# igilitschenski/multi_car_racing

Hardware: AMD Instinct MI355X
Metric: env-steps/sec (num_agents=2, 96x96 RGB obs) at batch=4096; 1 GPU (higher is better)
Workload: dtype f32 rigid-body state / f64 tyre model / u8 pixels

## Files before the change

### include/mcr.h

```cpp
#ifndef MCR_H
#define MCR_H
#include <stddef.h>
#include <stdint.h>
#ifdef __cplusplus
extern "C" {
#endif

#define MCR_OK 0
#define MCR_ERR_ARG (-1)
#define MCR_ERR_HIP (-2)
#define MCR_ERR_STATE (-3)
#define MCR_ERR_CAPACITY (-4)

#define MCR_MAX_AGENTS 8
#define MCR_TILE_CAP 512
#define MCR_QUAD_CAP 768
#define MCR_OBS_H 96
#define MCR_OBS_W 96
#define MCR_MT_WORDS 625
#define MCR_OBS_RGB 0
#define MCR_OBS_GRAY 1
#define MCR_OBS_STACK_MAX 8

typedef struct mcr_env mcr_env;
// ... 140 lines not shown
int mcr_debug_read_view_scratch(mcr_env* h, int view, void* out, int nbytes);
int mcr_debug_read_dynamics_stamps(mcr_env* h, uint64_t* out, int n_u64);
int mcr_debug_read_counters(mcr_env* h, uint64_t* out4);
int mcr_debug_read_counters8(mcr_env* h, uint64_t* out8);
int mcr_debug_read_verdict_mismatches(mcr_env* h, uint64_t* out1);
int mcr_concurrent_collide(const mcr_env* h);
int mcr_step_ordering(const mcr_env* h);
int mcr_step_ordering_for(const mcr_env* h, void* stream);
int mcr_bind_stream(mcr_env* h, void* stream);
int mcr_debug_read_env_records(mcr_env* h, void* out, int n_bytes);
int mcr_debug_read_partition(mcr_env* h, uint8_t* part_out, int32_t* clist_out);
int mcr_debug_next_verdicts(mcr_env* h, int fill_value, uint8_t* out_or_null);
int mcr_debug_read_contact_counts(mcr_env* h, int32_t* out );
int mcr_debug_read_contacts(mcr_env* h, uint32_t* out );
int mcr_debug_read_tile_touch(mcr_env* h, uint32_t* out );
int mcr_debug_read_proxy_ids(mcr_env* h, int env, int32_t* out, int cap);
int mcr_status(mcr_env* h, uint32_t* out, int n_words);
int mcr_debug_overlap(mcr_env* h, int n, const float* quads, const float* poses, int fixture, uint8_t* out);
int mcr_debug_level_stats(const uint8_t* d_done, const uint8_t* d_trunc ,
                          const double* d_ep_return , const int32_t* d_ep_len,
                          const int32_t* d_level, int num_envs, int num_agents, int K,
                          int32_t* d_finished , double* d_stats , void* stream);
int mcr_debug_contact_obs(const uint32_t* d_store, int num_envs, int num_agents, int accumulate,
                          int32_t* d_mask , double* d_impulse , void* stream);
#define MCR_TIMING_SLOTS 8
int mcr_timing_read(mcr_env* h, double* ms_out , int64_t* launches_out );

#ifdef __cplusplus
}
#endif
// ... 2 lines not shown
```

### multi_car_racing_amd/_lib.py

```python
import ctypes, os
import numpy as np

HERE = os.path.dirname(os.path.abspath(__file__))
LIB_PATH = os.environ.get("MCR_LIB_PATH") or os.path.join(HERE, "_lib", "libmcr_hip.so")

MAX_AGENTS = 8
TILE_CAP = 512
QUAD_CAP = 768
MT_WORDS = 625
OBS_RGB, OBS_GRAY, OBS_STACK_MAX = 0, 1, 8
REPEAT_MAX = 16
RANGE_RAYS_MAX = 32
GRID_MAX = 64
GRID_ROAD, GRID_FRESH, GRID_TAKEN, GRID_CAR = 1, 2, 4, 8
DRV_PARAMS = 10
DRIVER_PARAM_NAMES = ("L1", "L2", "v_max", "K_s", "K_c", "K_g", "K_b", "offset", "gas_max", "brake_max")
DRIVER_DEFAULTS = dict(zip(DRIVER_PARAM_NAMES, (4.0, 12.0, 70.0, 8.0, 20.0, 0.2, 0.1, 0.0, 1.0, 0.8)))
RC_PARAMS = 8
RACECRAFT_PARAM_NAMES = ("look", "w_block", "w_pass", "off_max", "d_safe", "K_f", "w_off", "v_off")
RACECRAFT_DEFAULTS = dict(zip(RACECRAFT_PARAM_NAMES, (24.0, 3.5, 4.25, 4.5, 16.0, 2.0, 7.5, 15.0)))
LEVEL_ORDER = {"random": 0, "cycle": 1}

DEBUG_VIEW_CLOCKS = 1 << 5
DEBUG_POS_ITERS_2 = 1 << 6
# ... 94 lines not shown
    "mcr_hull_polygons": (_i, [_vp, _vp]),
    "mcr_driver_defaults": (_i, [_vp]),
    "mcr_check_drivers": (_i, [_i, _vp, ctypes.c_uint32]),
    "mcr_set_drivers": (_i, [_vp, _vp, ctypes.c_uint32, _vp]),
    "mcr_driver_actions": (_i, [_vp, _vp, ctypes.c_uint32, _vp, _vp]),
    "mcr_racecraft_defaults": (_i, [_vp]),
    "mcr_check_racecraft": (_i, [_i, _vp, ctypes.c_uint32]),
    "mcr_set_racecraft": (_i, [_vp, _vp, ctypes.c_uint32]),
    "mcr_read_rollout_stats": (_i, [_vp, _vp, _i]),
    "mcr_render": (_i, [_vp, _i, _i, _i, _vp, _vp]),
    "mcr_debug_read_contact_counts": (_i, [_vp, _vp]),
    "mcr_debug_read_contacts": (_i, [_vp, _vp]),
    "mcr_debug_contact_obs": (_i, [_vp, _i, _i, _i, _vp, _vp, _vp]),
    "mcr_debug_read_tile_touch": (_i, [_vp, _vp]),
    "mcr_debug_read_proxy_ids": (_i, [_vp, _i, _vp, _i]),
    "mcr_debug_read_env_records": (_i, [_vp, _vp, _i]),
    "mcr_debug_read_partition": (_i, [_vp, _vp, _vp]),
    "mcr_debug_next_verdicts": (_i, [_vp, _i, _vp]),
    "mcr_debug_read_counters": (_i, [_vp, _vp]),
    "mcr_debug_read_counters8": (_i, [_vp, _vp]),
    "mcr_debug_read_verdict_mismatches": (_i, [_vp, _vp]),
    "mcr_concurrent_collide": (_i, [_vp]),
    "mcr_step_ordering": (_i, [_vp]),
    "mcr_step_ordering_for": (_i, [_vp, _vp]),
    "mcr_bind_stream": (_i, [_vp, _vp]),
    "mcr_debug_overlap": (_i, [_vp, _i, _vp, _vp, _i, _vp]),
    "mcr_debug_level_stats": (_i, [_vp, _vp, _vp, _vp, _vp, _i, _i, _i, _vp, _vp, _vp]),
    "mcr_status": (_i, [_vp, _vp, _i]),
    "mcr_world_create": (_vp, [_i]),
    "mcr_world_destroy": (None, [_vp]),
# ... 103 lines not shown
```

### multi_car_racing_amd/csrc/k_carview.h

```cpp
#pragma once
#include "mcr_kernels.h"

struct CarPose {
  float cx[5], cy[5], a[5];
  float hvx, hvy, hw;
  double omega[4], phase[4];
};
#define CARVIEW_ALL 31u
struct CarBox { float xl, yl, xh, yh; };

__device__ __forceinline__ CarPose car_pose_load(const float* __restrict__ carf, const double* __restrict__ card, const int stride, const int ci, const uint32_t parts) {
  CarPose c = {};
#pragma unroll
  for (int k = 0; k < 5; ++k) {
    const bool mine = (parts >> k) & 1u;
    if (mine) { c.cx[k] = carf[(CF_CX + k) * stride + ci]; c.cy[k] = carf[(CF_CY + k) * stride + ci]; }
    if (mine || (k == 1 && (parts & 1u))) c.a[k] = carf[(CF_A + k) * stride + ci];
    if (mine && k > 0) c.phase[k - 1] = card[(CD_PHASE + k - 1) * stride + ci];
  }
  if (parts & 1u) {
    c.hvx = carf[(CF_VX + 0) * stride + ci]; c.hvy = carf[(CF_VY + 0) * stride + ci]; c.hw = carf[(CF_W + 0) * stride + ci];
#pragma unroll
    for (int k = 0; k < 4; ++k) c.omega[k] = card[(CD_OMEGA + k) * stride + ci];
  }
  return c;
}
__device__ __forceinline__ void car_pose_store(float* __restrict__ carf, double* __restrict__ card, const int stride, const int ci, const CarPose& c) {
#pragma unroll
  for (int k = 0; k < 5; ++k) { carf[(CF_CX + k) * stride + ci] = c.cx[k]; carf[(CF_CY + k) * stride + ci] = c.cy[k]; carf[(CF_A + k) * stride + ci] = c.a[k]; }
  carf[(CF_VX + 0) * stride + ci] = c.hvx; carf[(CF_VY + 0) * stride + ci] = c.hvy; carf[(CF_W + 0) * stride + ci] = c.hw;
#pragma unroll
  for (int k = 0; k < 4; ++k) { card[(CD_OMEGA + k) * stride + ci] = c.omega[k]; card[(CD_PHASE + k) * stride + ci] = c.phase[k]; }
}

__device__ __forceinline__ void view_score(float* __restrict__ vp, const double reward_shown, const uint32_t flags) {
  vp[VP_SCORE] = __int_as_float(mcr_label_value(reward_shown));
  vp[VP_OLDFLAGS] = __uint_as_float(flags);
}

__device__ __forceinline__ void carbox_add(CarBox& box, const V2 v) {
// ... 21 lines not shown
    double s1, s2, c1, c2; mcr_sincos_core(a1, &s1, &c1); mcr_sincos_core(a2, &s2, &c2);
    int ns = 0;
    if (!(s1 > 0 && s2 > 0)) {
      if (s1 > 0) c1 = np_sign(c1);
      if (s2 > 0) c2 = np_sign(c2);
      ns = 4;
      const float lx[4] = {(float)(-MCR_WHEEL_W * MCR_SIZE), (float)(+MCR_WHEEL_W * MCR_SIZE), (float)(+MCR_WHEEL_W * MCR_SIZE), (float)(-MCR_WHEEL_W * MCR_SIZE)};
      const float ly[4] = {(float)(+MCR_WHEEL_R * c1 * MCR_SIZE), (float)(+MCR_WHEEL_R * c1 * MCR_SIZE), (float)(+MCR_WHEEL_R * c2 * MCR_SIZE), (float)(+MCR_WHEEL_R * c2 * MCR_SIZE)};
      V2 u[4];
#pragma unroll
      for (int i = 0; i < 4; ++i) u[i] = xmul(wxf, v2(lx[i], ly[i]));
      carpoly_quad(cp4 + (2 * k + 1) * 4, u);
    }
    *(float2*)(cnt + 2 * k) = make_float2(__int_as_float(S.wheel.n), __int_as_float(ns));
  }
  if (parts & 1u) {
    const Xf hxf = xf_of(v2(c.cx[0], c.cy[0]), c.a[0], v2(S.hull_lcx, S.hull_lcy));
    const double zoom = 0.1 * MCR_SCALE * fmax(1 - t, 0.0) + MCR_ZOOM * MCR_SCALE * fmin(t, 1.0);
    const double sx = (double)hxf.p.x, sy = (double)hxf.p.y;
    double angle = -(double)c.a[0];
    const double vx = (double)c.hvx, vy = (double)c.hvy;
    const double speed = sqrt(vx * vx + vy * vy);
    if (speed > 0.5) angle = atan2(vx, vy);
    double sin_a, cos_a; mcr_sincos_core(angle, &sin_a, &cos_a);
    const double ttx = MCR_WINDOW_W / 2 - (sx * zoom * cos_a - sy * zoom * sin_a);
    const double tty = MCR_WINDOW_H * h_ratio - (sx * zoom * sin_a + sy * zoom * cos_a);
    const float ftx = (float)ttx, fty = (float)tty, fz = (float)zoom;
    const float fdeg = (float)(57.29577951308232 * angle);
    const double rad = (double)fdeg * (3.14159265358979323846 / 180.0);
    double sin_r, cos_r; mcr_sincos_core(rad, &sin_r, &cos_r);
    const float fcs = (float)cos_r, fsn = (float)sin_r;
    const float kx = 96.0f / 1000.0f, ky = 96.0f / 800.0f;
    vp[VP_CAM + 0] = fcs * fz * kx; vp[VP_CAM + 1] = -fsn * fz * kx; vp[VP_CAM + 2] = fsn * fz * ky; vp[VP_CAM + 3] = fcs * fz * ky;
    vp[VP_CAM + 4] = ftx * kx; vp[VP_CAM + 5] = fty * ky;
    const float inv_z = 1.0f / fz;
    const float i0 = fcs * (1000.0f / 96.0f) * inv_z, i1 = fsn * (800.0f / 96.0f) * inv_z, i2 = -(fcs * ftx + fsn * fty) * inv_z;
    const float i3 = -fsn * (1000.0f / 96.0f) * inv_z, i4 = fcs * (800.0f / 96.0f) * inv_z, i5 = (fsn * ftx - fcs * fty) * inv_z;
    vp[VP_INV + 0] = i0; vp[VP_INV + 1] = i1; vp[VP_INV + 2] = i2; vp[VP_INV + 3] = i3; vp[VP_INV + 4] = i4; vp[VP_INV + 5] = i5;
    const double sW = MCR_WINDOW_W / 40.0, hH = MCR_WINDOW_H / 40.0;
    const double vals[5] = {0.02 * speed, 0.01 * c.omega[0], 0.01 * c.omega[1], 0.01 * c.omega[2], 0.01 * c.omega[3]};
    const double places[5] = {5, 7, 8, 9, 10};
    float hud_top = 12.0f;
#pragma unroll
    for (int i = 0; i < 5; ++i) {
      const float ya = (float)(hH + hH * vals[i]) * ky, yb = (float)hH * ky;
      vp[VP_IND + i * 4 + 0] = (float)((places[i] + 0) * sW) * kx; vp[VP_IND + i * 4 + 1] = (float)((places[i] + 1) * sW) * kx;
      vp[VP_IND + i * 4 + 2] = fminf(ya, yb); vp[VP_IND + i * 4 + 3] = fmaxf(ya, yb);
      hud_top = fmaxf(hud_top, fmaxf(ya, yb) + 1.0f);
    }
    const double jang = (double)(c.a[1] - c.a[0]);
    const double hv[2] = {-10.0 * jang, -0.8 * (double)c.hw};
    const double hp[2] = {20, 30};
#pragma unroll
    for (int i = 0; i < 2; ++i) {
      const float xa = (float)((hp[i] + 0) * sW) * kx, xb = (float)((hp[i] + hv[i]) * sW) * kx;
      vp[VP_IND + (5 + i) * 4 + 0] = fminf(xa, xb); vp[VP_IND + (5 + i) * 4 + 1] = fmaxf(xa, xb);
      vp[VP_IND + (5 + i) * 4 + 2] = (float)(2 * hH) * ky; vp[VP_IND + (5 + i) * 4 + 3] = (float)(4 * hH) * ky;
    }
    vp[VP_HUDTOP] = hud_top;
    {
      const float hk = 0.5f / (float)(MCR_PLAYFIELD / 20.0);
      const float aU = i0 * hk, bU = i1 * hk, cU = i2 * hk;
      const float aV = i3 * hk, bV = i4 * hk, cV = i5 * hk;
      float umin = MCR_MAXFLT, umax = -MCR_MAXFLT, vmin = MCR_MAXFLT, vmax = -MCR_MAXFLT;
#pragma unroll
      for (int k = 0; k < 4; ++k) {
        const float X = (k & 1) ? 96.0f : 0.0f, Y = (k & 2) ? 96.0f : 12.0f;
        const float u = aU * X + bU * Y + cU, v = aV * X + bV * Y + cV;
        umin = fminf(umin, u); umax = fmaxf(umax, u); vmin = fminf(vmin, v); vmax = fmaxf(vmax, v);
      }
      const float mu = fabsf(aU) + fabsf(bU) + 1e-3f, mv = fabsf(aV) + fabsf(bV) + 1e-3f;
      const bool inside_field = umin - mu >= -10.0f && umax + mu <= 10.0f && vmin - mv >= -10.0f && vmax + mv <= 10.0f;
      int a0 = (int)ceilf(umin - mu - 0.5f), a1 = (int)floorf(umax + mu), b0 = (int)ceilf(vmin - mv - 0.5f), b1 = (int)floorf(vmax + mv);
      a0 = max(a0, -10); a1 = min(a1, 9); b0 = max(b0, -10); b1 = min(b1, 9);
      vp[VP_GRASS + 0] = __int_as_float(a0); vp[VP_GRASS + 1] = __int_as_float(max(a1 - a0 + 1, 0));
      vp[VP_GRASS + 2] = __int_as_float(b0); vp[VP_GRASS + 3] = __int_as_float(max(b1 - b0 + 1, 0));
      vp[VP_GRASS + 4] = __int_as_float(inside_field ? 1 : 0);
    }
    int hn[4];
#pragma unroll
    for (int k = 0; k < 4; ++k) {
      const int n = hn[k] = __builtin_amdgcn_readfirstlane(S.hull[k].n);
      V2 w[8];
#pragma unroll
      for (int i = 0; i < 8; ++i) { if (i < n) w[i] = xmul(hxf, v2(S.hull[k].vx[i], S.hull[k].vy[i])); else w[i] = w[i - 1 < 0 ? 0 : i - 1]; }
#pragma unroll
      for (int i = 0; i < 8; ++i) carbox_add(box, w[i]);
      float4* hp4 = cp4 + (8 + k) * 4;
#pragma unroll
      for (int i = 0; i < 4; ++i) hp4[i] = make_float4(w[2 * i].x, w[2 * i].y, w[2 * i + 1].x, w[2 * i + 1].y);
    }
    *(float4*)(cnt + 8) = make_float4(__int_as_float(hn[0]), __int_as_float(hn[1]), __int_as_float(hn[2]), __int_as_float(hn[3]));
  }
  return box;
}
```

### multi_car_racing_amd/csrc/k_list_chain.h

```cpp
#pragma once
#include "k_collide.h"
#include "k_dynamics.h"
#include "k_flags.h"
#include "k_viewprep.h"

__device__ __forceinline__ void list_reset_pass(const McrParams& p, const int blk) {
  __threadfence();
  if (p.term_idx) for (int k = 0; k < p.list_envs_per_block; ++k) term_prepare(p, mcr_env_of_slot(p, blk * p.list_envs_per_block + k));
  for (int k = 0; k < p.list_envs_per_block; ++k) { collide_block(p, 1, blk * p.list_envs_per_block + k); __syncthreads(); }
  __threadfence();
  __syncthreads();
  dynamics_block<true>(p, 1, blk);
  __syncthreads();
}

template <bool CC>
__global__ __launch_bounds__(64) void k_list_chain(McrParams pa, McrParams pb, const int with_flags, const int ga) {
  __builtin_amdgcn_s_setprio(3);
  if (pa.role == ROLE_CONTACT && blockIdx.x == 0 && threadIdx.x == 0) __hip_atomic_store(&pa.host_counts[HC_CONTACT_ENVS], (uint32_t)pa.clist[0], __ATOMIC_RELAXED, __HIP_MEMORY_SCOPE_SYSTEM);
  if (pa.soft_sync && pa.role == ROLE_DEFERRED && pa.cc_mode) {
    if (threadIdx.x == 0) (void)mcr_await(pa, W_COL);
    __builtin_amdgcn_fence(__ATOMIC_ACQUIRE, "agent");
    __syncthreads();
  }
// ... 40 lines not shown
  for (int blk = blockIdx.x; blk < nb; blk += gridDim.x) flags_block(p, blk);
}

__global__ void k_term_finish(McrParams p) { term_finish(p); }
__global__ __launch_bounds__(64) void k_term_prep(McrParams p) { term_prepare(p, p.env0 + (int)blockIdx.x); }

__global__ void k_post(McrParams p, int w) {
  if (threadIdx.x == 0 && w == W_SIDE && p.fuse_collide) p.clist[0] = 0;
  if (threadIdx.x == 0 && !((p.debug & DEBUG_NO_SIDE_POST) && w == W_SIDE)) mcr_post(p, w);
}
__global__ void k_await(McrParams p, int w0, int w1) {
  if (threadIdx.x == 0) { if (w0 >= 0) (void)mcr_await(p, w0); if (w1 >= 0) (void)mcr_await(p, w1); }
}

__global__ __launch_bounds__(64) void k_viewprep_verdict(McrParams p, const int vp_blocks) {
  if ((int)blockIdx.x < vp_blocks) { viewprep_block(p, (int)blockIdx.x); return; }
  if (p.part_next == nullptr) return;
  const int env = mcr_env_of_slot(p, (int)blockIdx.x - vp_blocks);
  if (env >= p.env0 + p.nenv || p.part_next[env] != 2) return;
  verdict_block(p, env);
}
__global__ __launch_bounds__(64, 8) void k_flags_viewprep(McrParams p, const int vp_blocks) {
  if ((int)blockIdx.x < vp_blocks) viewprep_block(p, (int)blockIdx.x);
  else flags_block(p, (int)blockIdx.x - vp_blocks);
}
```

### multi_car_racing_amd/csrc/k_viewprep.h

```cpp
#pragma once
#include "k_carview.h"

__device__ __forceinline__ void viewprep_car(const McrShapes& S, const float* __restrict__ carf, const double* __restrict__ card, const int stride, const int ci,
                                             float* __restrict__ viewp, float* __restrict__ carpoly, const double h_ratio, const double t_now, const uint32_t parts = CARVIEW_ALL) {
  view_record(S, car_pose_load(carf, card, stride, ci, parts), t_now, h_ratio, viewp + (size_t)ci * MCR_VIEWP_FLOATS, carpoly + (size_t)ci * MCR_CARPOLY_FLOATS, parts);
}

__device__ __forceinline__ void viewprep_block(const McrParams& p, const int blk) {
  const int g = blk * 64 + threadIdx.x;
  const int env = mcr_env_of_slot(p, g / p.G), agent = g % p.G;
  if (env >= p.env0 + p.nenv || agent >= p.N) return;
  const McrEnvState es = p.env[env];
  if (!es.active || es.just_reset) return;
  viewprep_car(*p.shapes, p.carf, p.card, p.BN, env * p.N + agent, p.viewp, p.carpoly, p.h_ratio, es.t);
}
__device__ __forceinline__ void viewprep_list_block(const McrParams& p, const int blk) {
  if (p.obs == nullptr) return;
  __builtin_amdgcn_fence(__ATOMIC_SEQ_CST, "workgroup");
  const int lane = threadIdx.x & 63, ncars = p.list_envs_per_block * p.N;
  for (int base = 0; base < ncars * 8; base += 64) {
    const int w = base + lane, c = w >> 3, part = w & 7;
    if (c >= ncars || part >= 5) continue;
    const int env = mcr_env_of_slot(p, blk * p.list_envs_per_block + c / p.N);
    if (env >= p.env0 + p.nenv) continue;
    const McrEnvState es = p.env[env];
    if (!es.active || es.resetting) continue;
    viewprep_car(*p.shapes, p.carf, p.card, p.BN, env * p.N + c % p.N, p.viewp, p.carpoly, p.h_ratio, es.t, 1u << part);
  }
}
__device__ __forceinline__ void term_prepare(const McrParams& p, const int env) {
  if (p.term_idx == nullptr || env >= p.env0 + p.nenv) return;
  const McrEnvState es = p.env[env];
  if (!es.active || !es.resetting) return;
  const int tidx = p.term_idx[env];
  if (tidx < 0) return;
  const int lane = threadIdx.x & 63;
  const uint32_t* __restrict__ src = (const uint32_t*)(p.tile_flags + (size_t)env * MCR_TILE_CAP);
  uint32_t* __restrict__ dst = (uint32_t*)(p.term_tflags + (size_t)tidx * MCR_TILE_CAP);
  for (int i = lane; i < MCR_TILE_CAP / 2; i += 64) dst[i] = src[i];
  if (lane < p.N) viewprep_car(*p.shapes, p.term_carf, p.term_card, p.term_cap * p.N, tidx * p.N + lane, p.term_viewp, p.term_carpoly, p.h_ratio, p.term_env[tidx].t);
}
__global__ __launch_bounds__(64) void k_viewprep(McrParams p) { viewprep_block(p, (int)blockIdx.x); }
__global__ __launch_bounds__(64) void k_viewprep_now(McrParams p) {
  const int ci = (int)blockIdx.x * 64 + (int)threadIdx.x;
  if (ci >= p.BN) return;
  const McrEnvState es = p.env[ci / p.N];
  if (!es.active) return;
  viewprep_car(*p.shapes, p.carf, p.card, p.BN, ci, p.viewp, p.carpoly, p.h_ratio, es.t);
  view_score(p.viewp + (size_t)ci * MCR_VIEWP_FLOATS, p.card[CD_REWARD * p.BN + ci], p.caru[CU_FLAGS * p.BN + ci]);
}
```

### multi_car_racing_amd/csrc/mcr_debug.hip

```cpp
#define MCR_DEVICE_FUNCTIONS_ONLY
#include "mcr_env.h"
#include "k_collide.h"
#include "k_contactobs.h"
#include <algorithm>

__global__ void k_synth_actions(float* __restrict__ out, int n_cars, int N, unsigned long long seed, unsigned t, unsigned env_offset) {
  const int ci = blockIdx.x * blockDim.x + threadIdx.x;
  if (ci >= n_cars) return;
  float a[3];
  mcr_synth_action(seed, env_offset + (unsigned)(ci / N), (unsigned)(ci % N), t + blockIdx.y, a);
  float* o = out + ((size_t)blockIdx.y * n_cars + ci) * 3;
  o[0] = a[0]; o[1] = a[1]; o[2] = a[2];
}
extern "C" int mcr_synth_actions_block(mcr_env* h, float* d_actions, uint64_t seed, uint32_t t0, int nsteps, uint32_t env_offset, void* stream) {
  if (!h || !d_actions || nsteps < 1 || nsteps > 65535) { g_err = "bad argument"; return MCR_ERR_ARG; }
  hipLaunchKernelGGL(k_synth_actions, dim3((h->P.BN + 255) / 256, nsteps), dim3(256), 0, (hipStream_t)stream, d_actions, h->P.BN, h->P.N,
                     (unsigned long long)seed, t0, env_offset);
  HIPCHK(hipGetLastError());
  return MCR_OK;
}
extern "C" int mcr_synth_actions(mcr_env* h, float* d_actions, uint64_t seed, uint32_t t, uint32_t env_offset, void* stream) {
  return mcr_synth_actions_block(h, d_actions, seed, t, 1, env_offset, stream);
}

// ... 69 lines not shown
  HIPCHK(hipDeviceSynchronize());
  const size_t stride = MCR_CC_MAX * MCR_CC_WORDS + 4;
  HIPCHK(hipMemcpy2D(out, sizeof(int32_t), h->P.cc_store, stride * sizeof(uint32_t), sizeof(int32_t), h->cfg.num_envs, hipMemcpyDeviceToHost));
  return MCR_OK;
}
extern "C" int mcr_debug_read_contacts(mcr_env* h, uint32_t* out) {
  if (!h || !out) return MCR_ERR_ARG;
  return read_back(out, h->P.cc_store, sizeof(uint32_t) * MCR_CC_STORE_WORDS * (size_t)h->cfg.num_envs);
}
extern "C" int mcr_debug_read_tile_touch(mcr_env* h, uint32_t* out) {
  if (!h || !out) { g_err = "mcr_debug_read_tile_touch: null argument"; return MCR_ERR_ARG; }
  HIPCHK(sync_state(h));
  HIPCHK(hipMemcpy(out, h->P.tile_touch, sizeof(uint32_t) * MCR_TILE_CAP * (size_t)h->cfg.num_envs, hipMemcpyDeviceToHost));
  return MCR_OK;
}
extern "C" int mcr_debug_read_proxy_ids(mcr_env* h, int env, int32_t* out, int cap) {
  if (!h || !out || env < 0 || env >= h->cfg.num_envs) return MCR_ERR_ARG;
  if (!h->P.pid_tab) { g_err = "mcr_debug_read_proxy_ids: the handle was created with fresh_world = 1 (ids ascend in creation order)"; return MCR_ERR_STATE; }
  HIPCHK(hipDeviceSynchronize());
  std::vector<uint16_t> tab(MCR_PID_TAB); int32_t meta[4];
  HIPCHK(hipMemcpy(tab.data(), h->P.pid_tab + (size_t)env * MCR_PID_TAB, sizeof(uint16_t) * MCR_PID_TAB, hipMemcpyDeviceToHost));
  HIPCHK(hipMemcpy(meta, h->P.pid_meta + (size_t)env * 4, sizeof(meta), hipMemcpyDeviceToHost));
  const int T = meta[2], F = 8 * h->cfg.num_agents;
  int n = 0;
  for (int t = 0; t < T && n < cap; ++t) out[n++] = tab[t];
  for (int f = 0; f < F && n < cap; ++f) out[n++] = tab[MCR_TILE_CAP + f];
  return n;
}
extern "C" int mcr_debug_read_dynamics_stamps(mcr_env* h, uint64_t* out, int n_u64) {
  if (!h || !out) return MCR_ERR_ARG;
// ... 65 lines not shown
```

### multi_car_racing_amd/csrc/mcr_hip.hip

```cpp
#include "mcr_env.h"
#include "k_dynamics.h"
#include "k_collide.h"
#include "k_raster_common.h"
#include "k_flags.h"
#include "k_viewprep.h"
#include "k_list_chain.h"
#include "k_render.h"
#include <hip/hip_ext.h>
#include <cstring>
#include <cstdlib>

thread_local std::string g_err;
extern "C" const char* mcr_last_error(void) { return g_err.c_str(); }
extern "C" const char* mcr_version(void) { return "mcr-hip 0.1 (gfx950)"; }

#define MCR_LIST_GRID 128
static bool cc_active(const mcr_env* h) { return h->split && h->concurrent_collide; }

#include <mutex>
#include <algorithm>
static std::mutex g_soft_mu;
static std::vector<mcr_env*> g_soft_list;

__global__ void k_probe_wait(int* flag, int* result) {
// ... 324 lines not shown
  StepGrids g;
  g.dyn_blocks = mcr_dyn_blocks(B, P.G);
  g.lg_con = std::min(B, 2 * h->chain_grid);
  g.prev_contacts = std::min(B, (int)((volatile uint32_t*)h->status_host)[MCR_STATUS_WORDS + HC_CONTACT_ENVS]);
  g.lg_flags = std::min(B * N, (N <= 2 ? 4 : 32) * MCR_LIST_GRID);
  g.ga = std::min({(B + MCR_SIDE_ENVS_PER_WAVE - 1) / MCR_SIDE_ENVS_PER_WAVE, h->chain_grid, MCR_LIST_GRID / 2});
  g.gb = P.auto_reset ? std::min(B, MCR_LIST_GRID) : 0;
  g.vg_con = std::min(2048, g.prev_contacts * N + g.prev_contacts * N / 4 + 8);
  return g;
}

static void step_phase_words(mcr_env* h, const McrParams& Pin, const StepGrids& g, hipStream_t st, int view_flags) {
  const int B = Pin.B, N = Pin.N, dyn_blocks = g.dyn_blocks;
  const bool draw = Pin.obs != nullptr, cc = Pin.cc_mode != 0;
  const int vif = (view_flags && draw && h->viewprep_in_flags) ? 1 : 0;
  const bool defer_flags = vif && cc && g.prev_contacts <= 64 && !(Pin.debug & DEBUG_FLAGS_IN_STEP);
  const bool take_flags = cc && h->flags_pending;
  const McrParams P = with(Pin, ROLE_MAIN, [&](McrParams& q) { q.soft_sync = 1; q.flags_deferred = take_flags ? 1 : 0; q.split = 0; q.viewprep_in_flags = vif; });
  const McrParams Pbegin = with(P, ROLE_ALL, [](McrParams& q) { q.split = 1; q.viewprep_in_flags = 0; });
  const McrParams Pside = with(P, ROLE_CONTACT, [](McrParams& q) { q.viewprep_in_flags = 0; });
  if (!cc) LAUNCH_LDS(0, k_collide, B, 64, col::lds_bytes(N), st, Pbegin, 0);
  if (h->flags_pending && !cc) flush_flags(h, st);
  LAUNCH(1, k_dynamics<false>, dyn_blocks, 64, st, with(P, ROLE_MAIN), 0);
  hipLaunchKernelGGL(k_await, dim3(1), dim3(64), 0, h->s_side, Pbegin, (int)W_BEGIN, -1);
  if (cc) {
    hipLaunchKernelGGL(k_await, dim3(1), dim3(64), 0, h->s_defer, Pbegin, (int)W_BEGIN, -1);
    if (take_flags) flush_flags(h, h->s_defer);
    LAUNCH_LDS(0, k_collide, B, 64, col::lds_bytes(N), h->s_defer, Pbegin, 0);
    hipLaunchKernelGGL(k_post, dim3(1), dim3(64), 0, h->s_defer, Pbegin, (int)W_COL);
  }
  { const McrParams Pc = with(Pside, ROLE_CONTACT, [](McrParams& q) { q.list_envs_per_block = 1; }); LAUNCH_LDS(5, k_list_chain<true>, g.lg_con, 64, col::lds_bytes(N), h->s_side, Pc, Pc, 0, g.lg_con); }
  const int fiv = (view_flags && draw && N <= 8) ? (N <= 2 ? 8 : 64) : 0;
  const int fiv_c = fiv ? std::min(512, std::max(fiv, (g.prev_contacts * (N + 1) + 3) / 4 + 2)) : 0;
  if (view_flags && !fiv) hipLaunchKernelGGL(k_flags_list, dim3(g.lg_flags), dim3(64), 0, h->s_side, Pside);
  if (draw) launch_view(h, 6, P.term_cnt ? 2 * B : B, h->s_side, with(Pside, ROLE_CONTACT, [&](McrParams& q) { q.flags_blocks = fiv_c; }), 0, nullptr, g.vg_con);
  hipLaunchKernelGGL(k_post, dim3(1), dim3(64), 0, h->s_side, Pside, (int)W_SIDE);
  const bool flags_on_caller = view_flags && draw && !vif && N <= 7;
  LAUNCH_LDS(7, k_list_chain<false>, g.ga + g.gb, 64, col::lds_bytes(N), st, with(P, ROLE_DEFERRED), with(P, ROLE_RESPAWN, [](McrParams& q) { q.list_envs_per_block = 1; }), 0, g.ga);
  if (view_flags && !fiv) hipLaunchKernelGGL(k_flags_list, dim3(g.lg_flags), dim3(64), 0, st, with(P, ROLE_DEFERRED));
  if (flags_on_caller) launch_flags(st, with(P, ROLE_MAIN));
  if (draw) launch_view(h, 7, P.term_cnt ? 2 * B : B, st, with(P, P.auto_reset ? ROLE_DEFERRED_RESPAWN : ROLE_DEFERRED, [&](McrParams& q) { q.await_tail = 1; q.flags_blocks = fiv; }), 0);
  hipLaunchKernelGGL(k_await, dim3(1), dim3(64), 0, h->s_defer, with(P, ROLE_MAIN), (int)W_DYN, -1);
  if (defer_flags) {
    hipLaunchKernelGGL(k_viewprep_verdict, dim3(dyn_blocks + B), dim3(64), 0, h->s_defer, with(P, ROLE_MAIN), dyn_blocks);
    h->flags_P = with(P, ROLE_MAIN, [](McrParams& q) { q.part_next = nullptr; q.flags_deferred = 0; }); h->flags_pending = true;
  }
  else if (vif) hipLaunchKernelGGL(k_flags_viewprep, dim3(dyn_blocks + B * N), dim3(64), 0, h->s_defer, with(P, ROLE_MAIN), dyn_blocks);
  else if (view_flags && !flags_on_caller) launch_flags(h->s_defer, with(P, ROLE_MAIN));
  if (draw) launch_view(h, 2, B, h->s_defer, with(P, ROLE_MAIN, [](McrParams& q) { q.use_vorder = 1; }), 0);
  hipLaunchKernelGGL(k_post, dim3(1), dim3(64), 0, h->s_defer, with(P, ROLE_MAIN), (int)W_MAIN);
  if (!draw) hipLaunchKernelGGL(k_await, dim3(1), dim3(64), 0, st, with(P, ROLE_MAIN), (int)W_SIDE, (int)W_MAIN);
}

static void step_events(mcr_env* h, const McrParams& Pin, const StepGrids& g, hipStream_t st, int view_flags) {
  const int B = Pin.B, N = Pin.N, dyn_blocks = g.dyn_blocks;
  const bool draw = Pin.obs != nullptr, cc = Pin.cc_mode != 0;
  const bool sev = h->use_graph <= 0 && !capturing(st);
  const int vif = (view_flags && draw && h->viewprep_in_flags) ? 1 : 0;
  const McrParams P = with(Pin, ROLE_MAIN, [&](McrParams& q) { q.split = 0; q.viewprep_in_flags = vif; });
  const McrParams Pbegin = with(P, ROLE_ALL, [](McrParams& q) { q.split = 1; q.viewprep_in_flags = 0; });
  const McrParams Pside = with(P, ROLE_CONTACT, [](McrParams& q) { q.viewprep_in_flags = 0; });
#define STOP(ev) (sev ? (ev) : (hipEvent_t) nullptr)
// ... 6 lines not shown
  const int fuse_flags = (view_flags && N <= 2) ? 1 : 0;
  const bool flags_list = view_flags && !fuse_flags;
  { const McrParams Pc = with(Pside, ROLE_CONTACT, [](McrParams& q) { q.list_envs_per_block = 1; }); LAUNCH_LDS_STOP(5, k_list_chain<true>, g.lg_con, 64, col::lds_bytes(N), h->s_side, STOP((!draw && !flags_list) ? h->ev_join : nullptr), Pc, Pc, fuse_flags, g.lg_con); }
  if (flags_list) hipExtLaunchKernelGGL(k_flags_list, dim3(g.lg_flags), dim3(64), 0, h->s_side, nullptr, STOP(!draw ? h->ev_join : nullptr), 0, Pside);
  if (draw) launch_view(h, 6, P.term_cnt ? 2 * B : B, h->s_side, Pside, 0, STOP(h->ev_join), g.vg_con);
  LAUNCH_LDS_STOP(1, k_dynamics<false>, dyn_blocks, 64, 0, st, STOP(h->ev_fork2), with(P, ROLE_MAIN), 0);
  RECORD_UNLESS_STOP(h->ev_fork2, st);
  (void)hipStreamWaitEvent(h->s_defer, h->ev_fork2, 0);
  (void)hipStreamWaitEvent(st, h->ev_col, 0);
  if (!draw) (void)hipStreamWaitEvent(h->s_side, h->ev_fork2, 0);
  LAUNCH_LDS(7, k_list_chain<false>, g.ga + g.gb, 64, col::lds_bytes(N), st, with(P, ROLE_DEFERRED), with(P, ROLE_RESPAWN, [](McrParams& q) { q.list_envs_per_block = 1; }), fuse_flags, g.ga);
  if (flags_list) hipLaunchKernelGGL(k_flags_list, dim3(g.lg_flags), dim3(64), 0, st, with(P, ROLE_DEFERRED));
  if (draw) launch_view(h, 7, P.term_cnt ? 2 * B : B, st, with(P, P.auto_reset ? ROLE_DEFERRED_RESPAWN : ROLE_DEFERRED), 0);
  RECORD_UNLESS_STOP(h->ev_join, h->s_side);
  const hipEvent_t main_done = h->ev_join2;
  if (vif) hipLaunchKernelGGL(k_viewprep, dim3(dyn_blocks), dim3(64), 0, h->s_defer, with(P, ROLE_MAIN));
  if (view_flags) hipExtLaunchKernelGGL(k_flags, dim3(B * N), dim3(64), 0, h->s_defer, nullptr, STOP(!draw ? main_done : nullptr), 0, with(P, ROLE_MAIN));
  (void)hipStreamWaitEvent(h->s_defer, h->ev_col, 0);
  if (draw) launch_view(h, 2, B, h->s_defer, with(P, ROLE_MAIN, [](McrParams& q) { q.use_vorder = 1; }), 0, STOP(main_done));
  if (!sev || (!draw && !view_flags)) (void)hipEventRecord(h->ev_join2, h->s_defer);
  (void)hipStreamWaitEvent(st, h->ev_join, 0);
  (void)hipStreamWaitEvent(st, h->ev_join2, 0);
  if (P.term_cnt) hipLaunchKernelGGL(k_term_finish, dim3(1), dim3(256), 0, st, with(P, ROLE_MAIN));
#undef STOP
#undef RECORD_UNLESS_STOP
}

static void launch_step(mcr_env* h, McrParams P, hipStream_t st, int view_flags) {
  step_prologue(h, P, st);
  if (!h->split) { step_single_stream(h, P, st, view_flags); return; }
  P.defer_after = MCR_DEFER_AFTER; P.respawn_list = P.auto_reset ? 1 : 0; P.list_envs_per_block = MCR_SIDE_ENVS_PER_WAVE;
// ... 235 lines not shown
```

### multi_car_racing_amd/csrc/mcr_kernels.h

```cpp
#pragma once
#include "mcr_common.h"

struct McrTermEnv { double t; int32_t slot, env, consumed, pad; };

enum McrRole { ROLE_ALL = 0, ROLE_MAIN = 1, ROLE_CONTACT = 2, ROLE_DEFERRED = 3, ROLE_RESPAWN = 4, ROLE_DEFERRED_RESPAWN = 5, ROLE_TERMINAL = 6 };
#define mcr_is_list_role(role) ((role) >= ROLE_CONTACT)
#define mcr_is_main_role(role) ((role) < ROLE_CONTACT)

enum McrDebugBit {
  DEBUG_VIEW_CLOCKS        = 1 << 5,
  DEBUG_POS_ITERS_2        = 1 << 6,
  DEBUG_VEL_ITERS_2        = 1 << 7,
  DEBUG_DYN_CLOCKS         = 1 << 8,
  DEBUG_NO_CC_VELOCITY     = 1 << 9,
  DEBUG_NO_CC_EXCHANGE     = 1 << 10,
  DEBUG_EPOCH_ACQ_REL      = 1 << 11,
  DEBUG_STARVED_COLLIDE    = 1 << 12,
  DEBUG_SHORT_AWAIT        = DEBUG_STARVED_COLLIDE,
  DEBUG_SHORT_EPOCH_WAIT   = DEBUG_STARVED_COLLIDE,
  DEBUG_WITHHOLD_ENV0_EPOCH = DEBUG_STARVED_COLLIDE,
  DEBUG_NO_SIDE_POST       = 1 << 13,
  DEBUG_OLD_SOLVE_ORDER    = 1 << 14,
  DEBUG_COLLIDE_CLOCKS     = 1 << 15,
  DEBUG_DYN_CLOCKS_VEL     = 1 << 16,
  DEBUG_TRACE              = 1 << 17,
  DEBUG_SLOW_COLLIDE       = 1 << 18,
  DEBUG_FLAGS_IN_STEP      = 1 << 19,
  DEBUG_DROP_PENDING_FLAGS = 1 << 20,
};
__host__ __device__ __forceinline__ int mcr_dyn_blocks(int B, int G) { return (B * G + 63) / 64; }

struct McrParams {
  int32_t B, N, G;
  int32_t BN;
  int32_t env0, nenv;
  float* carf;
  double* card;
  uint32_t* caru;
  McrEnvState* env;
  uint8_t* slots;
  uint32_t* tile_touch;
  uint16_t* tile_flags;
  uint32_t* cc_store;
  float4* bpf;
  uint32_t* cc_stamp;
// ... 245 lines not shown
```

Baseline: 19.27 million.

## Split view-record preparation into seven per-part blocks (camera, wheels, HUD, hull)

```diff
diff --git a/include/mcr.h b/include/mcr.h
--- a/include/mcr.h
+++ b/include/mcr.h
@@ -178,6 +178,7 @@
 int mcr_debug_read_contact_counts(mcr_env* h, int32_t* out );
 int mcr_debug_read_contacts(mcr_env* h, uint32_t* out );
 int mcr_debug_read_tile_touch(mcr_env* h, uint32_t* out );
+int mcr_debug_read_view_records(mcr_env* h, float* viewp_out , float* carpoly_out );
 int mcr_debug_read_proxy_ids(mcr_env* h, int env, int32_t* out, int cap);
 int mcr_status(mcr_env* h, uint32_t* out, int n_words);
 int mcr_debug_overlap(mcr_env* h, int n, const float* quads, const float* poses, int fixture, uint8_t* out);
diff --git a/multi_car_racing_amd/_lib.py b/multi_car_racing_amd/_lib.py
--- a/multi_car_racing_amd/_lib.py
+++ b/multi_car_racing_amd/_lib.py
@@ -132,6 +132,7 @@
     "mcr_debug_contact_obs": (_i, [_vp, _i, _i, _i, _vp, _vp, _vp]),
     "mcr_debug_read_tile_touch": (_i, [_vp, _vp]),
     "mcr_debug_read_proxy_ids": (_i, [_vp, _i, _vp, _i]),
+    "mcr_debug_read_view_records": (_i, [_vp, _vp, _vp]),
     "mcr_debug_read_env_records": (_i, [_vp, _vp, _i]),
     "mcr_debug_read_partition": (_i, [_vp, _vp, _vp]),
     "mcr_debug_next_verdicts": (_i, [_vp, _i, _vp]),
diff --git a/multi_car_racing_amd/csrc/k_carview.h b/multi_car_racing_amd/csrc/k_carview.h
--- a/multi_car_racing_amd/csrc/k_carview.h
+++ b/multi_car_racing_amd/csrc/k_carview.h
@@ -6,24 +6,43 @@
   float hvx, hvy, hw;
   double omega[4], phase[4];
 };
-#define CARVIEW_ALL 31u
+#define CARVIEW_CAMERA 1u
+#define CARVIEW_WHEEL(k) (2u << (k))
+#define CARVIEW_HUD 32u
+#define CARVIEW_HULL 64u
+#define CARVIEW_BODY (CARVIEW_CAMERA | CARVIEW_HUD | CARVIEW_HULL)
+#define CARVIEW_ALL 127u
 struct CarBox { float xl, yl, xh, yh; };
 
 __device__ __forceinline__ CarPose car_pose_load(const float* __restrict__ carf, const double* __restrict__ card, const int stride, const int ci, const uint32_t parts) {
   CarPose c = {};
+  const bool hud = (parts & CARVIEW_HUD) != 0;
 #pragma unroll
   for (int k = 0; k < 5; ++k) {
-    const bool mine = (parts >> k) & 1u;
+    const bool mine = k == 0 ? (parts & (CARVIEW_CAMERA | CARVIEW_HULL)) != 0 : ((parts >> k) & 1u) != 0;
     if (mine) { c.cx[k] = carf[(CF_CX + k) * stride + ci]; c.cy[k] = carf[(CF_CY + k) * stride + ci]; }
-    if (mine || (k == 1 && (parts & 1u))) c.a[k] = carf[(CF_A + k) * stride + ci];
+    if (mine || (k <= 1 && hud)) c.a[k] = carf[(CF_A + k) * stride + ci];
     if (mine && k > 0) c.phase[k - 1] = card[(CD_PHASE + k - 1) * stride + ci];
   }
-  if (parts & 1u) {
-    c.hvx = carf[(CF_VX + 0) * stride + ci]; c.hvy = carf[(CF_VY + 0) * stride + ci]; c.hw = carf[(CF_W + 0) * stride + ci];
+  if (parts & (CARVIEW_CAMERA | CARVIEW_HUD)) { c.hvx = carf[(CF_VX + 0) * stride + ci]; c.hvy = carf[(CF_VY + 0) * stride + ci]; }
+  if (hud) {
+    c.hw = carf[(CF_W + 0) * stride + ci];
 #pragma unroll
     for (int k = 0; k < 4; ++k) c.omega[k] = card[(CD_OMEGA + k) * stride + ci];
   }
   return c;
+}
+__device__ __forceinline__ void car_pose_pin(CarPose& c, const uint32_t parts) {
+  const bool hud = (parts & CARVIEW_HUD) != 0;
+#pragma unroll
+  for (int k = 0; k < 5; ++k) {
+    const bool mine = k == 0 ? (parts & (CARVIEW_CAMERA | CARVIEW_HULL)) != 0 : ((parts >> k) & 1u) != 0;
+    if (mine) asm volatile("" : "+v"(c.cx[k]), "+v"(c.cy[k]));
+    if (mine || (k <= 1 && hud)) asm volatile("" : "+v"(c.a[k]));
+    if (mine && k > 0) asm volatile("" : "+v"(c.phase[k - 1]));
+  }
+  if (parts & (CARVIEW_CAMERA | CARVIEW_HUD)) asm volatile("" : "+v"(c.hvx), "+v"(c.hvy));
+  if (hud) asm volatile("" : "+v"(c.hw), "+v"(c.omega[0]), "+v"(c.omega[1]), "+v"(c.omega[2]), "+v"(c.omega[3]));
 }
 __device__ __forceinline__ void car_pose_store(float* __restrict__ carf, double* __restrict__ card, const int stride, const int ci, const CarPose& c) {
 #pragma unroll
@@ -75,51 +94,57 @@
     }
     *(float2*)(cnt + 2 * k) = make_float2(__int_as_float(S.wheel.n), __int_as_float(ns));
   }
-  if (parts & 1u) {
+  if (parts & CARVIEW_BODY) {
+    const bool cam = (parts & CARVIEW_CAMERA) != 0, hud = (parts & CARVIEW_HUD) != 0, hull = (parts & CARVIEW_HULL) != 0;
     const Xf hxf = xf_of(v2(c.cx[0], c.cy[0]), c.a[0], v2(S.hull_lcx, S.hull_lcy));
-    const double zoom = 0.1 * MCR_SCALE * fmax(1 - t, 0.0) + MCR_ZOOM * MCR_SCALE * fmin(t, 1.0);
-    const double sx = (double)hxf.p.x, sy = (double)hxf.p.y;
-    double angle = -(double)c.a[0];
     const double vx = (double)c.hvx, vy = (double)c.hvy;
     const double speed = sqrt(vx * vx + vy * vy);
-    if (speed > 0.5) angle = atan2(vx, vy);
-    double sin_a, cos_a; mcr_sincos_core(angle, &sin_a, &cos_a);
-    const double ttx = MCR_WINDOW_W / 2 - (sx * zoom * cos_a - sy * zoom * sin_a);
-    const double tty = MCR_WINDOW_H * h_ratio - (sx * zoom * sin_a + sy * zoom * cos_a);
-    const float ftx = (float)ttx, fty = (float)tty, fz = (float)zoom;
-    const float fdeg = (float)(57.29577951308232 * angle);
-    const double rad = (double)fdeg * (3.14159265358979323846 / 180.0);
-    double sin_r, cos_r; mcr_sincos_core(rad, &sin_r, &cos_r);
-    const float fcs = (float)cos_r, fsn = (float)sin_r;
     const float kx = 96.0f / 1000.0f, ky = 96.0f / 800.0f;
-    vp[VP_CAM + 0] = fcs * fz * kx; vp[VP_CAM + 1] = -fsn * fz * kx; vp[VP_CAM + 2] = fsn * fz * ky; vp[VP_CAM + 3] = fcs * fz * ky;
-    vp[VP_CAM + 4] = ftx * kx; vp[VP_CAM + 5] = fty * ky;
-    const float inv_z = 1.0f / fz;
-    const float i0 = fcs * (1000.0f / 96.0f) * inv_z, i1 = fsn * (800.0f / 96.0f) * inv_z, i2 = -(fcs * ftx + fsn * fty) * inv_z;
-    const float i3 = -fsn * (1000.0f / 96.0f) * inv_z, i4 = fcs * (800.0f / 96.0f) * inv_z, i5 = (fsn * ftx - fcs * fty) * inv_z;
-    vp[VP_INV + 0] = i0; vp[VP_INV + 1] = i1; vp[VP_INV + 2] = i2; vp[VP_INV + 3] = i3; vp[VP_INV + 4] = i4; vp[VP_INV + 5] = i5;
-    const double sW = MCR_WINDOW_W / 40.0, hH = MCR_WINDOW_H / 40.0;
-    const double vals[5] = {0.02 * speed, 0.01 * c.omega[0], 0.01 * c.omega[1], 0.01 * c.omega[2], 0.01 * c.omega[3]};
-    const double places[5] = {5, 7, 8, 9, 10};
-    float hud_top = 12.0f;
+    float i0 = 0.0f, i1 = 0.0f, i2 = 0.0f, i3 = 0.0f, i4 = 0.0f, i5 = 0.0f;
+    if (cam) {
+      const double zoom = 0.1 * MCR_SCALE * fmax(1 - t, 0.0) + MCR_ZOOM * MCR_SCALE * fmin(t, 1.0);
+      const double sx = (double)hxf.p.x, sy = (double)hxf.p.y;
+      double angle = -(double)c.a[0];
+      if (speed > 0.5) angle = atan2(vx, vy);
+      double sin_a, cos_a; mcr_sincos_core(angle, &sin_a, &cos_a);
+      const double ttx = MCR_WINDOW_W / 2 - (sx * zoom * cos_a - sy * zoom * sin_a);
+      const double tty = MCR_WINDOW_H * h_ratio - (sx * zoom * sin_a + sy * zoom * cos_a);
+      const float ftx = (float)ttx, fty = (float)tty, fz = (float)zoom;
+      const float fdeg = (float)(57.29577951308232 * angle);
+      const double rad = (double)fdeg * (3.14159265358979323846 / 180.0);
+      double sin_r, cos_r; mcr_sincos_core(rad, &sin_r, &cos_r);
+      const float fcs = (float)cos_r, fsn = (float)sin_r;
+      vp[VP_CAM + 0] = fcs * fz * kx; vp[VP_CAM + 1] = -fsn * fz * kx; vp[VP_CAM + 2] = fsn * fz * ky; vp[VP_CAM + 3] = fcs * fz * ky;
+      vp[VP_CAM + 4] = ftx * kx; vp[VP_CAM + 5] = fty * ky;
+      const float inv_z = 1.0f / fz;
+      i0 = fcs * (1000.0f / 96.0f) * inv_z; i1 = fsn * (800.0f / 96.0f) * inv_z; i2 = -(fcs * ftx + fsn * fty) * inv_z;
+      i3 = -fsn * (1000.0f / 96.0f) * inv_z; i4 = fcs * (800.0f / 96.0f) * inv_z; i5 = (fsn * ftx - fcs * fty) * inv_z;
+      vp[VP_INV + 0] = i0; vp[VP_INV + 1] = i1; vp[VP_INV + 2] = i2; vp[VP_INV + 3] = i3; vp[VP_INV + 4] = i4; vp[VP_INV + 5] = i5;
+    }
+    if (hud) {
+      const double sW = MCR_WINDOW_W / 40.0, hH = MCR_WINDOW_H / 40.0;
+      const double vals[5] = {0.02 * speed, 0.01 * c.omega[0], 0.01 * c.omega[1], 0.01 * c.omega[2], 0.01 * c.omega[3]};
+      const double places[5] = {5, 7, 8, 9, 10};
+      float hud_top = 12.0f;
 #pragma unroll
-    for (int i = 0; i < 5; ++i) {
-      const float ya = (float)(hH + hH * vals[i]) * ky, yb = (float)hH * ky;
-      vp[VP_IND + i * 4 + 0] = (float)((places[i] + 0) * sW) * kx; vp[VP_IND + i * 4 + 1] = (float)((places[i] + 1) * sW) * kx;
-      vp[VP_IND + i * 4 + 2] = fminf(ya, yb); vp[VP_IND + i * 4 + 3] = fmaxf(ya, yb);
-      hud_top = fmaxf(hud_top, fmaxf(ya, yb) + 1.0f);
+      for (int i = 0; i < 5; ++i) {
+        const float ya = (float)(hH + hH * vals[i]) * ky, yb = (float)hH * ky;
+        vp[VP_IND + i * 4 + 0] = (float)((places[i] + 0) * sW) * kx; vp[VP_IND + i * 4 + 1] = (float)((places[i] + 1) * sW) * kx;
+        vp[VP_IND + i * 4 + 2] = fminf(ya, yb); vp[VP_IND + i * 4 + 3] = fmaxf(ya, yb);
+        hud_top = fmaxf(hud_top, fmaxf(ya, yb) + 1.0f);
+      }
+      const double jang = (double)(c.a[1] - c.a[0]);
+      const double hv[2] = {-10.0 * jang, -0.8 * (double)c.hw};
+      const double hp[2] = {20, 30};
+#pragma unroll
+      for (int i = 0; i < 2; ++i) {
+        const float xa = (float)((hp[i] + 0) * sW) * kx, xb = (float)((hp[i] + hv[i]) * sW) * kx;
+        vp[VP_IND + (5 + i) * 4 + 0] = fminf(xa, xb); vp[VP_IND + (5 + i) * 4 + 1] = fmaxf(xa, xb);
+        vp[VP_IND + (5 + i) * 4 + 2] = (float)(2 * hH) * ky; vp[VP_IND + (5 + i) * 4 + 3] = (float)(4 * hH) * ky;
+      }
+      vp[VP_HUDTOP] = hud_top;
     }
-    const double jang = (double)(c.a[1] - c.a[0]);
-    const double hv[2] = {-10.0 * jang, -0.8 * (double)c.hw};
-    const double hp[2] = {20, 30};
-#pragma unroll
-    for (int i = 0; i < 2; ++i) {
-      const float xa = (float)((hp[i] + 0) * sW) * kx, xb = (float)((hp[i] + hv[i]) * sW) * kx;
-      vp[VP_IND + (5 + i) * 4 + 0] = fminf(xa, xb); vp[VP_IND + (5 + i) * 4 + 1] = fmaxf(xa, xb);
-      vp[VP_IND + (5 + i) * 4 + 2] = (float)(2 * hH) * ky; vp[VP_IND + (5 + i) * 4 + 3] = (float)(4 * hH) * ky;
-    }
-    vp[VP_HUDTOP] = hud_top;
-    {
+    if (cam) {
       const float hk = 0.5f / (float)(MCR_PLAYFIELD / 20.0);
       const float aU = i0 * hk, bU = i1 * hk, cU = i2 * hk;
       const float aV = i3 * hk, bV = i4 * hk, cV = i5 * hk;
@@ -138,20 +163,22 @@
       vp[VP_GRASS + 2] = __int_as_float(b0); vp[VP_GRASS + 3] = __int_as_float(max(b1 - b0 + 1, 0));
       vp[VP_GRASS + 4] = __int_as_float(inside_field ? 1 : 0);
     }
-    int hn[4];
+    if (hull) {
+      int hn[4];
 #pragma unroll
-    for (int k = 0; k < 4; ++k) {
-      const int n = hn[k] = __builtin_amdgcn_readfirstlane(S.hull[k].n);
-      V2 w[8];
+      for (int k = 0; k < 4; ++k) {
+        const int n = hn[k] = __builtin_amdgcn_readfirstlane(S.hull[k].n);
+        V2 w[8];
 #pragma unroll
-      for (int i = 0; i < 8; ++i) { if (i < n) w[i] = xmul(hxf, v2(S.hull[k].vx[i], S.hull[k].vy[i])); else w[i] = w[i - 1 < 0 ? 0 : i - 1]; }
+        for (int i = 0; i < 8; ++i) { if (i < n) w[i] = xmul(hxf, v2(S.hull[k].vx[i], S.hull[k].vy[i])); else w[i] = w[i - 1 < 0 ? 0 : i - 1]; }
 #pragma unroll
-      for (int i = 0; i < 8; ++i) carbox_add(box, w[i]);
-      float4* hp4 = cp4 + (8 + k) * 4;
+        for (int i = 0; i < 8; ++i) carbox_add(box, w[i]);
+        float4* hp4 = cp4 + (8 + k) * 4;
 #pragma unroll
-      for (int i = 0; i < 4; ++i) hp4[i] = make_float4(w[2 * i].x, w[2 * i].y, w[2 * i + 1].x, w[2 * i + 1].y);
+        for (int i = 0; i < 4; ++i) hp4[i] = make_float4(w[2 * i].x, w[2 * i].y, w[2 * i + 1].x, w[2 * i + 1].y);
+      }
+      *(float4*)(cnt + 8) = make_float4(__int_as_float(hn[0]), __int_as_float(hn[1]), __int_as_float(hn[2]), __int_as_float(hn[3]));
     }
-    *(float4*)(cnt + 8) = make_float4(__int_as_float(hn[0]), __int_as_float(hn[1]), __int_as_float(hn[2]), __int_as_float(hn[3]));
   }
   return box;
 }
diff --git a/multi_car_racing_amd/csrc/k_list_chain.h b/multi_car_racing_amd/csrc/k_list_chain.h
--- a/multi_car_racing_amd/csrc/k_list_chain.h
+++ b/multi_car_racing_amd/csrc/k_list_chain.h
@@ -78,13 +78,13 @@
 }
 
 __global__ __launch_bounds__(64) void k_viewprep_verdict(McrParams p, const int vp_blocks) {
-  if ((int)blockIdx.x < vp_blocks) { viewprep_block(p, (int)blockIdx.x); return; }
+  if ((int)blockIdx.x < vp_blocks) { viewprep_parts_block(p, (int)blockIdx.x); return; }
   if (p.part_next == nullptr) return;
   const int env = mcr_env_of_slot(p, (int)blockIdx.x - vp_blocks);
   if (env >= p.env0 + p.nenv || p.part_next[env] != 2) return;
   verdict_block(p, env);
 }
 __global__ __launch_bounds__(64, 8) void k_flags_viewprep(McrParams p, const int vp_blocks) {
-  if ((int)blockIdx.x < vp_blocks) viewprep_block(p, (int)blockIdx.x);
+  if ((int)blockIdx.x < vp_blocks) viewprep_parts_block(p, (int)blockIdx.x);
   else flags_block(p, (int)blockIdx.x - vp_blocks);
 }
diff --git a/multi_car_racing_amd/csrc/k_viewprep.h b/multi_car_racing_amd/csrc/k_viewprep.h
--- a/multi_car_racing_amd/csrc/k_viewprep.h
+++ b/multi_car_racing_amd/csrc/k_viewprep.h
@@ -6,13 +6,34 @@
   view_record(S, car_pose_load(carf, card, stride, ci, parts), t_now, h_ratio, viewp + (size_t)ci * MCR_VIEWP_FLOATS, carpoly + (size_t)ci * MCR_CARPOLY_FLOATS, parts);
 }
 
-__device__ __forceinline__ void viewprep_block(const McrParams& p, const int blk) {
-  const int g = blk * 64 + threadIdx.x;
-  const int env = mcr_env_of_slot(p, g / p.G), agent = g % p.G;
+template <uint32_t PARTS>
+__device__ __forceinline__ void viewprep_part(const McrParams& p, const int env, const int ci) {
+  const bool marks = p.role == ROLE_MAIN;
+  uint32_t m_contact = marks ? p.part[env] : 0u, m_deferred = marks ? p.dpart[env] : 0u;
+  const McrEnvState* __restrict__ E = p.env + env;
+  double t_now = E->t;
+  int active = E->active, just_reset = E->just_reset;
+  CarPose c = car_pose_load(p.carf, p.card, p.BN, ci, PARTS);
+  asm volatile("" : "+v"(m_contact), "+v"(m_deferred), "+v"(active), "+v"(just_reset), "+v"(t_now));
+  car_pose_pin(c, PARTS);
+  if (m_contact | m_deferred) return;
+  if (!active || just_reset) return;
+  view_record(*p.shapes, c, t_now, p.h_ratio, p.viewp + (size_t)ci * MCR_VIEWP_FLOATS, p.carpoly + (size_t)ci * MCR_CARPOLY_FLOATS, PARTS);
+}
+__device__ __forceinline__ void viewprep_parts_block(const McrParams& p, const int blk) {
+  const int part = blk % CARVIEW_NPARTS, g = (blk / CARVIEW_NPARTS) * 64 + (int)threadIdx.x;
+  const int env = p.env0 + g / p.G, agent = g % p.G;
   if (env >= p.env0 + p.nenv || agent >= p.N) return;
-  const McrEnvState es = p.env[env];
-  if (!es.active || es.just_reset) return;
-  viewprep_car(*p.shapes, p.carf, p.card, p.BN, env * p.N + agent, p.viewp, p.carpoly, p.h_ratio, es.t);
+  const int ci = env * p.N + agent;
+  switch (part) {
+    case 0: viewprep_part<CARVIEW_CAMERA>(p, env, ci); break;
+    case 1: viewprep_part<CARVIEW_WHEEL(0)>(p, env, ci); break;
+    case 2: viewprep_part<CARVIEW_WHEEL(1)>(p, env, ci); break;
+    case 3: viewprep_part<CARVIEW_WHEEL(2)>(p, env, ci); break;
+    case 4: viewprep_part<CARVIEW_WHEEL(3)>(p, env, ci); break;
+    case 5: viewprep_part<CARVIEW_HUD>(p, env, ci); break;
+    default: viewprep_part<CARVIEW_HULL>(p, env, ci); break;
+  }
 }
 __device__ __forceinline__ void viewprep_list_block(const McrParams& p, const int blk) {
   if (p.obs == nullptr) return;
@@ -25,7 +46,7 @@
     if (env >= p.env0 + p.nenv) continue;
     const McrEnvState es = p.env[env];
     if (!es.active || es.resetting) continue;
-    viewprep_car(*p.shapes, p.carf, p.card, p.BN, env * p.N + c % p.N, p.viewp, p.carpoly, p.h_ratio, es.t, 1u << part);
+    viewprep_car(*p.shapes, p.carf, p.card, p.BN, env * p.N + c % p.N, p.viewp, p.carpoly, p.h_ratio, es.t, part == 0 ? CARVIEW_BODY : 1u << part);
   }
 }
 __device__ __forceinline__ void term_prepare(const McrParams& p, const int env) {
@@ -40,7 +61,7 @@
   for (int i = lane; i < MCR_TILE_CAP / 2; i += 64) dst[i] = src[i];
   if (lane < p.N) viewprep_car(*p.shapes, p.term_carf, p.term_card, p.term_cap * p.N, tidx * p.N + lane, p.term_viewp, p.term_carpoly, p.h_ratio, p.term_env[tidx].t);
 }
-__global__ __launch_bounds__(64) void k_viewprep(McrParams p) { viewprep_block(p, (int)blockIdx.x); }
+__global__ __launch_bounds__(64) void k_viewprep(McrParams p) { viewprep_parts_block(p, (int)blockIdx.x); }
 __global__ __launch_bounds__(64) void k_viewprep_now(McrParams p) {
   const int ci = (int)blockIdx.x * 64 + (int)threadIdx.x;
   if (ci >= p.BN) return;
diff --git a/multi_car_racing_amd/csrc/mcr_debug.hip b/multi_car_racing_amd/csrc/mcr_debug.hip
--- a/multi_car_racing_amd/csrc/mcr_debug.hip
+++ b/multi_car_racing_amd/csrc/mcr_debug.hip
@@ -107,6 +107,14 @@
   HIPCHK(hipMemcpy(out, h->P.tile_touch, sizeof(uint32_t) * MCR_TILE_CAP * (size_t)h->cfg.num_envs, hipMemcpyDeviceToHost));
   return MCR_OK;
 }
+extern "C" int mcr_debug_read_view_records(mcr_env* h, float* viewp_out, float* carpoly_out) {
+  if (!h || !viewp_out || !carpoly_out) { g_err = "mcr_debug_read_view_records: null argument"; return MCR_ERR_ARG; }
+  HIPCHK(sync_state(h));
+  const size_t BN = (size_t)h->cfg.num_envs * h->cfg.num_agents;
+  HIPCHK(hipMemcpy(viewp_out, h->P.viewp, sizeof(float) * MCR_VIEWP_FLOATS * BN, hipMemcpyDeviceToHost));
+  HIPCHK(hipMemcpy(carpoly_out, h->P.carpoly, sizeof(float) * MCR_CARPOLY_FLOATS * BN, hipMemcpyDeviceToHost));
+  return MCR_OK;
+}
 extern "C" int mcr_debug_read_proxy_ids(mcr_env* h, int env, int32_t* out, int cap) {
   if (!h || !out || env < 0 || env >= h->cfg.num_envs) return MCR_ERR_ARG;
   if (!h->P.pid_tab) { g_err = "mcr_debug_read_proxy_ids: the handle was created with fresh_world = 1 (ids ascend in creation order)"; return MCR_ERR_STATE; }
diff --git a/multi_car_racing_amd/csrc/mcr_hip.hip b/multi_car_racing_amd/csrc/mcr_hip.hip
--- a/multi_car_racing_amd/csrc/mcr_hip.hip
+++ b/multi_car_racing_amd/csrc/mcr_hip.hip
@@ -362,6 +362,7 @@
   const int B = Pin.B, N = Pin.N, dyn_blocks = g.dyn_blocks;
   const bool draw = Pin.obs != nullptr, cc = Pin.cc_mode != 0;
   const int vif = (view_flags && draw && h->viewprep_in_flags) ? 1 : 0;
+  const int vp_blocks = mcr_viewprep_blocks(B, Pin.G);
   const bool defer_flags = vif && cc && g.prev_contacts <= 64 && !(Pin.debug & DEBUG_FLAGS_IN_STEP);
   const bool take_flags = cc && h->flags_pending;
   const McrParams P = with(Pin, ROLE_MAIN, [&](McrParams& q) { q.soft_sync = 1; q.flags_deferred = take_flags ? 1 : 0; q.split = 0; q.viewprep_in_flags = vif; });
@@ -390,10 +391,10 @@
   if (draw) launch_view(h, 7, P.term_cnt ? 2 * B : B, st, with(P, P.auto_reset ? ROLE_DEFERRED_RESPAWN : ROLE_DEFERRED, [&](McrParams& q) { q.await_tail = 1; q.flags_blocks = fiv; }), 0);
   hipLaunchKernelGGL(k_await, dim3(1), dim3(64), 0, h->s_defer, with(P, ROLE_MAIN), (int)W_DYN, -1);
   if (defer_flags) {
-    hipLaunchKernelGGL(k_viewprep_verdict, dim3(dyn_blocks + B), dim3(64), 0, h->s_defer, with(P, ROLE_MAIN), dyn_blocks);
+    hipLaunchKernelGGL(k_viewprep_verdict, dim3(vp_blocks + B), dim3(64), 0, h->s_defer, with(P, ROLE_MAIN), vp_blocks);
     h->flags_P = with(P, ROLE_MAIN, [](McrParams& q) { q.part_next = nullptr; q.flags_deferred = 0; }); h->flags_pending = true;
   }
-  else if (vif) hipLaunchKernelGGL(k_flags_viewprep, dim3(dyn_blocks + B * N), dim3(64), 0, h->s_defer, with(P, ROLE_MAIN), dyn_blocks);
+  else if (vif) hipLaunchKernelGGL(k_flags_viewprep, dim3(vp_blocks + B * N), dim3(64), 0, h->s_defer, with(P, ROLE_MAIN), vp_blocks);
   else if (view_flags && !flags_on_caller) launch_flags(h->s_defer, with(P, ROLE_MAIN));
   if (draw) launch_view(h, 2, B, h->s_defer, with(P, ROLE_MAIN, [](McrParams& q) { q.use_vorder = 1; }), 0);
   hipLaunchKernelGGL(k_post, dim3(1), dim3(64), 0, h->s_defer, with(P, ROLE_MAIN), (int)W_MAIN);
@@ -430,7 +431,7 @@
   if (draw) launch_view(h, 7, P.term_cnt ? 2 * B : B, st, with(P, P.auto_reset ? ROLE_DEFERRED_RESPAWN : ROLE_DEFERRED), 0);
   RECORD_UNLESS_STOP(h->ev_join, h->s_side);
   const hipEvent_t main_done = h->ev_join2;
-  if (vif) hipLaunchKernelGGL(k_viewprep, dim3(dyn_blocks), dim3(64), 0, h->s_defer, with(P, ROLE_MAIN));
+  if (vif) hipLaunchKernelGGL(k_viewprep, dim3(mcr_viewprep_blocks(B, P.G)), dim3(64), 0, h->s_defer, with(P, ROLE_MAIN));
   if (view_flags) hipExtLaunchKernelGGL(k_flags, dim3(B * N), dim3(64), 0, h->s_defer, nullptr, STOP(!draw ? main_done : nullptr), 0, with(P, ROLE_MAIN));
   (void)hipStreamWaitEvent(h->s_defer, h->ev_col, 0);
   if (draw) launch_view(h, 2, B, h->s_defer, with(P, ROLE_MAIN, [](McrParams& q) { q.use_vorder = 1; }), 0, STOP(main_done));
diff --git a/multi_car_racing_amd/csrc/mcr_kernels.h b/multi_car_racing_amd/csrc/mcr_kernels.h
--- a/multi_car_racing_amd/csrc/mcr_kernels.h
+++ b/multi_car_racing_amd/csrc/mcr_kernels.h
@@ -29,6 +29,8 @@
   DEBUG_DROP_PENDING_FLAGS = 1 << 20,
 };
 __host__ __device__ __forceinline__ int mcr_dyn_blocks(int B, int G) { return (B * G + 63) / 64; }
+#define CARVIEW_NPARTS 7
+__host__ __device__ __forceinline__ int mcr_viewprep_blocks(int B, int G) { return mcr_dyn_blocks(B, G) * CARVIEW_NPARTS; }
 
 struct McrParams {
   int32_t B, N, G;
```

Result: no change. 19.17 million (-0.5%).
